# k-xlsx/huff-encoding

Hardware: AMD Instinct MI355X
Metric: encode+decode GB/s on 1 GiB bytes at 1/2/4/8 MI355X; % HBM roofline (higher is better)
Workload: dtype u8; 1 GPU; 1 GiB uniform bytes (BASELINE configs[1]), encode+decode, bit-exact; bytes_per_gpu=1073741824, global_bytes=1073741824, compressed_bytes_per_gpu=1073741824, parallelism=shard1

## Files before the change

### huff-encoding_amd/csrc/device/pack.hip

```cpp
#include "pack_emit.hpp"

namespace huff::dev {

namespace {

template <bool LONG>
constexpr int pack_waves() { return LONG ? 4 : static_cast<int>(kPackWaves); }
#ifndef HUFF_PACK_BPL
#define HUFF_PACK_BPL 16
#endif
#ifndef HUFF_PACK_AHEAD
#define HUFF_PACK_AHEAD 2
#endif
constexpr uint32_t kBPL = HUFF_PACK_BPL;
constexpr uint32_t kRoundB = 64 * kBPL;
constexpr int kAhead = HUFF_PACK_AHEAD;
static_assert(kBPL % 16 == 0, "lanes load whole 16-byte pieces");
static_assert(kBPL <= kIdx && kTaskSym % kRoundB == 0, "an index entry starts a lane; a task is whole rounds");
constexpr int kPieces = kBPL / 16;

struct LaneIn {
    uint4 v[kPieces];
};

#ifndef HUFF_PACK_COPIES
#define HUFF_PACK_COPIES 32
#endif
constexpr int kCopies = HUFF_PACK_COPIES;
template <bool LONG>
constexpr uint32_t table_words() { return 256u * kCopies * (LONG ? 2u : 1u); }

template <bool LONG, int G = 1>
__global__ __launch_bounds__(pack_waves<LONG>() * 64) void k_pack(PackArgs a) {
    constexpr int kWaves = pack_waves<LONG>();
    constexpr int kThreads = kWaves * 64;
    constexpr int C = kCopies;
    constexpr int LOGC = C == 32 ? 5 : C == 16 ? 4 : C == 8 ? 3 : -1;
    static_assert(LOGC > 0, "8, 16 or 32 table copies");
    using E = Entry<LONG>;
    using T = typename E::T;
    extern __shared__ __attribute__((aligned(16))) uint32_t lds[];
    T* tab = reinterpret_cast<T*>(lds);
    const uint32_t t = threadIdx.x, lane = t & 63, copy = t & (C - 1), wave = wave_index();
    uint32_t* stage = lds + table_words<LONG>() + wave * a.stage_words;

    const T* tg = reinterpret_cast<const T*>(LONG ? static_cast<const void*>(a.table.l) : static_cast<const void*>(a.table.s));
#pragma unroll 4
    for (int i = 0; i < 256 / (kThreads / C); ++i) {
        const uint32_t e = (t >> LOGC) + (kThreads / C) * i;
        tab[(e << LOGC) | copy] = tg[e];
    }
    for (uint32_t i = lane; i < a.stage_words; i += 64) stage[i] = 0;
    __syncthreads();

    for (uint32_t c = blockIdx.x * kWaves + wave; c < a.nchunks; c += a.grid * kWaves) {
        const uint64_t sym0 = static_cast<uint64_t>(c) * kChunk;
        const uint64_t nsym = (a.n - sym0 < kChunk) ? a.n - sym0 : kChunk;
        const uint64_t prev8 = (lane == 0 && sym0 >= 8) ? *reinterpret_cast<const uint64_t*>(a.in + sym0 - 8) : 0;
        const uint64_t cs = a.chunk_start[c];
        const uint64_t ce = a.chunk_start[c + 1];
        uint64_t stage_bit0 = (cs >> 7) << 7;
        const uint64_t own_lo = cs >> 3;
        const uint64_t own_hi = (c + 1 == a.nchunks) ? (ce + 7) >> 3 : ce >> 3;
        const uint32_t nrounds = static_cast<uint32_t>((nsym + kRoundB - 1) / kRoundB);
        const auto rin = buf_rsrc(a.in + sym0, static_cast<uint32_t>((nsym + 15) & ~15ull));

        auto load_round = [&](uint32_t r) {
            LaneIn x;
#pragma unroll
            for (int q = 0; q < kPieces; ++q) x.v[q] = buf_ld16(rin, r * kRoundB + lane * kBPL + 16 * q);
            return x;
        };
        LaneIn vq[kAhead];
#pragma unroll
        for (int i = 0; i < kAhead; ++i) vq[i] = load_round(i);

        if (lane == 0 && (cs & 7)) {
            const int64_t floor8 = static_cast<int64_t>(cs & ~7ull);
            int64_t pos = static_cast<int64_t>(cs);
            for (uint32_t k = 1; k <= 8 && pos > floor8; ++k) {
                uint8_t b;
                if (sym0 >= k) {
                    b = static_cast<uint8_t>(prev8 >> (8 * (8 - k)));
                } else {
                    const uint32_t j = k - static_cast<uint32_t>(sym0);
                    if (j > a.prev_tail_len) break;
                    b = a.prev_tail[8 - j];
                }
                const T ent = tab[static_cast<uint32_t>(b) << LOGC];
                const int64_t len = static_cast<int64_t>(ent & E::kMask);
                const uint64_t code = E::code(ent);
                if (len == 0) break;
                const int64_t start = pos - len;
                for (int64_t q = (start > floor8 ? start : floor8); q < pos; ++q) {
                    if ((code >> (pos - 1 - q)) & 1) {
                        const uint64_t sb = static_cast<uint64_t>(q) - stage_bit0;
                        stage[sb >> 5] |= 0x80000000u >> (sb & 31);
                    }
                }
                pos = start;
            }
        }
        wave_sync();

        uint64_t round_bit = cs, task_bit0 = cs;
        constexpr uint32_t kRoundsPerTask = kTaskSym / kRoundB;
        for (uint32_t r = 0; r < nrounds; ++r) {
            const LaneIn v = vq[0];
#pragma unroll
            for (int i = 0; i + 1 < kAhead; ++i) vq[i] = vq[i + 1];
            vq[kAhead - 1] = load_round(r + kAhead);
            const uint32_t s_in_chunk = r * kRoundB + lane * kBPL;
            const uint32_t nsym32 = static_cast<uint32_t>(nsym);
            const int nvalid = s_in_chunk >= nsym32 ? 0
                                                    : static_cast<int>(nsym32 - s_in_chunk < kBPL ? nsym32 - s_in_chunk : kBPL);

            uint32_t bits = 0;
            uint32_t wv[4 * kPieces];
#pragma unroll
            for (int q = 0; q < kPieces; ++q) {
                wv[4 * q] = v.v[q].x;
                wv[4 * q + 1] = v.v[q].y;
                wv[4 * q + 2] = v.v[q].z;
                wv[4 * q + 3] = v.v[q].w;
            }
            T ent[kBPL];
            auto lookup = [&](int k) -> T { return tab[(((wv[k >> 2] >> (8 * (k & 3))) & 0xFFu) << LOGC) | copy]; };
            if ((r + 1ull) * kRoundB <= nsym) {
#pragma unroll
                for (int k = 0; k < static_cast<int>(kBPL); ++k) ent[k] = lookup(k);
            } else {
#pragma unroll
                for (int k = 0; k < static_cast<int>(kBPL); ++k) ent[k] = (k < nvalid) ? lookup(k) : T(0);
            }
            uint32_t Lp[kBPL / 2];
            if constexpr (!LONG && G >= 2) {
#pragma unroll
                for (int k = 0; k < static_cast<int>(kBPL / 2); ++k) {
                    Lp[k] = len2(static_cast<uint32_t>(ent[2 * k]), static_cast<uint32_t>(ent[2 * k + 1]));
                    bits += Lp[k];
                }
            } else {
#pragma unroll
                for (int k = 0; k < static_cast<int>(kBPL); ++k) bits += static_cast<uint32_t>(ent[k] & E::kMask);
            }
            const uint32_t incl = wave_scan_incl(bits);
            const uint32_t tot = static_cast<uint32_t>(__builtin_amdgcn_readlane(static_cast<int>(incl), 63));
            const uint32_t excl = incl - bits;

            if (a.sub16) {
                if ((r % kRoundsPerTask) == 0) {
                    task_bit0 = round_bit;
                    if (lane == 0) a.task_base[(sym0 + r * kRoundB) / kTaskSym] = round_bit;
                }
                if (nvalid > 0 && (s_in_chunk & (kIdx - 1)) == 0)
                    a.sub16[(sym0 + s_in_chunk) / kIdx] = static_cast<uint16_t>(round_bit - task_bit0 + excl);
            } else if (a.sub_bit && nvalid > 0 && (s_in_chunk & (kIdx - 1)) == 0) {
                a.sub_bit[(sym0 + s_in_chunk) / kIdx] = static_cast<uint32_t>(round_bit - cs + excl);
            }

            if constexpr (LONG) {
                if (bits) emit_codes<LONG, static_cast<int>(kBPL)>(stage, round_bit - stage_bit0 + excl, ent);
            } else {
                emit_codes_or<G>(stage, static_cast<uint32_t>(round_bit - stage_bit0 + excl), ent, Lp);
            }
            wave_order();

            const uint64_t end_bit = round_bit + tot;
            const bool last = (r + 1 == nrounds);
            const uint32_t nseg_done = static_cast<uint32_t>((end_bit - stage_bit0) >> 7);
            const uint32_t nseg_store = last ? static_cast<uint32_t>((end_bit - stage_bit0 + 127) >> 7) : nseg_done;
            const uint64_t sb0 = stage_bit0 >> 3;
            const uint32_t full_lo = own_lo > sb0 ? static_cast<uint32_t>((own_lo - sb0 + 15) >> 4) : 0u;
            const uint64_t hi_rel = own_hi > sb0 ? (own_hi - sb0) >> 4 : 0;
            const uint32_t full_hi = static_cast<uint32_t>(hi_rel < 0x7FFFFFFFull ? hi_rel : 0x7FFFFFFFull);
            for (uint32_t s = lane; s < nseg_store; s += 64)
                store_segment(stage, s, sb0 + 16ull * s, full_lo, full_hi, own_lo, own_hi, a.out);
            const uint32_t used_words = static_cast<uint32_t>((end_bit - stage_bit0 + 31) >> 5);
            uint32_t keep = 0;
            if (!last && lane < 4) keep = stage[nseg_done * 4 + lane];
            wave_order();
            for (uint32_t i = lane; i < (used_words + 3) / 4; i += 64)
                reinterpret_cast<uint4*>(stage)[i] = make_uint4(0, 0, 0, 0);
            wave_order();
            if (!last) {
                if (lane < 4) stage[lane] = keep;
                stage_bit0 += static_cast<uint64_t>(nseg_done) << 7;
                wave_order();
            }
            round_bit = end_bit;
        }
    }
}

}

size_t pack_lds_bytes(bool long_codes, uint32_t max_len, uint32_t stage_words) {
    (void)max_len;
    const uint32_t table = long_codes ? table_words<true>() : table_words<false>();
    const uint32_t waves = long_codes ? pack_waves<true>() : pack_waves<false>();
    return static_cast<size_t>(table + waves * stage_words) * 4;
}

uint32_t pack_round_bytes() { return kRoundB; }

uint32_t pack_waves_per_group(bool long_codes) { return long_codes ? pack_waves<true>() : pack_waves<false>(); }

namespace {
using PackKern = void (*)(PackArgs);
PackKern pack_kernel(bool long_codes, uint32_t max_len) {
    if (long_codes) return k_pack<true>;
    if (max_len <= 8) return k_pack<false, 4>;
    if (max_len <= 16) return k_pack<false, 2>;
    return k_pack<false, 1>;
}
}

uint32_t pack_groups_per_cu(bool long_codes, uint32_t max_len, size_t lds) {
    int per = 0;
    const int threads = (long_codes ? pack_waves<true>() : pack_waves<false>()) * 64;
    if (hipOccupancyMaxActiveBlocksPerMultiprocessor(&per, pack_kernel(long_codes, max_len), threads, lds) !=
            hipSuccess ||
        per < 1) {
        const size_t by_lds = lds ? (160 * 1024) / lds : 8;
        per = static_cast<int>(by_lds < 1 ? 1 : by_lds > 8 ? 8 : by_lds);
    }
    return static_cast<uint32_t>(per);
}

hipError_t launch_pack(bool long_codes, const PackArgs& a, hipStream_t s) {
    if (a.nchunks == 0) return hipSuccess;
    const size_t lds = pack_lds_bytes(long_codes, a.max_len, a.stage_words);
    launch_k(pack_kernel(long_codes, a.max_len), dim3(a.grid),
             dim3((long_codes ? pack_waves<true>() : pack_waves<false>()) * 64), lds, s, a);
    return hipGetLastError();
}

}
```

### huff-encoding_amd/csrc/device/pack_emit.hpp

```cpp
#pragma once

#include "bitreader.hpp"

namespace huff::dev {

template <bool LONG>
struct Entry;
template <>
struct Entry<false> {
    using T = uint32_t;
    static constexpr uint32_t kMask = 31;
    __device__ static uint64_t code(T e) {
        const uint32_t len = e & 31u;
        return len ? e >> (32 - len) : 0u;
    }
};
template <>
struct Entry<true> {
    using T = uint64_t;
    static constexpr uint32_t kMask = 63;
    __device__ static uint64_t code(T e) { return e >> 6; }
};

template <bool LONG, int N>
__device__ __forceinline__ void emit_codes(uint32_t* __restrict__ stage, uint64_t p,
                                           const typename Entry<LONG>::T (&ent)[N]) {
    using E = Entry<LONG>;
    uint32_t w = static_cast<uint32_t>(p >> 5);
    uint32_t nacc = static_cast<uint32_t>(p & 31);
    bool shared_first = nacc != 0;
    uint64_t acc = 0;
    auto flush = [&]() {
        if (nacc >= 32) {
            const uint32_t word = static_cast<uint32_t>(acc >> (nacc - 32));
            if (shared_first) {
                __hip_atomic_fetch_or(&stage[w], word, __ATOMIC_RELAXED, __HIP_MEMORY_SCOPE_WORKGROUP);
                shared_first = false;
            } else {
                stage[w] = word;
            }
            ++w;
            nacc -= 32;
        }
    };
#pragma unroll
    for (int k = 0; k < N; ++k) {
        const uint32_t len = static_cast<uint32_t>(ent[k] & E::kMask);
        const uint64_t code = E::code(ent[k]);
        if (LONG && len > 32) {
            const uint32_t hl = len - 32;
            acc = (acc << hl) | (code >> 32);
            nacc += hl;
            flush();
            acc = (acc << 32) | (code & 0xFFFFFFFFull);
            nacc += 32;
            flush();
        } else {
            acc = (acc << len) | code;
            nacc += len;
            flush();
        }
    }
    if (nacc) {
        const uint32_t word = static_cast<uint32_t>(acc << (32 - nacc));
        __hip_atomic_fetch_or(&stage[w], word, __ATOMIC_RELAXED, __HIP_MEMORY_SCOPE_WORKGROUP);
    }
}

__device__ __forceinline__ uint32_t join2(uint32_t e0, uint32_t e1) {
    return (e0 & ~31u) | ((e1 & ~31u) >> (e0 & 31u));
}

__device__ __forceinline__ uint32_t len2(uint32_t e0, uint32_t e1) {
    uint32_t r;
    asm("v_add_u32_sdwa %0, %1, %2 dst_sel:DWORD dst_unused:UNUSED_PAD src0_sel:BYTE_0 src1_sel:BYTE_0"
        : "=v"(r)
        : "v"(e0), "v"(e1));
    return r;
}

template <int G, int N>
__device__ __forceinline__ void emit_codes_or(uint32_t* __restrict__ stage, uint32_t p, const uint32_t (&ent)[N],
                                              const uint32_t (&Lp)[N / 2]) {
    const uint32_t stage_addr = static_cast<uint32_t>(reinterpret_cast<uintptr_t>(
        (__attribute__((address_space(3))) uint32_t*)(stage)));
    uint32_t o = p;
#pragma unroll
    for (int k = 0; k < N; k += G) {
        uint32_t J, len;
        if constexpr (G == 1) {
            J = ent[k] & ~31u;
            len = ent[k] & 31u;
        } else if constexpr (G == 2) {
            J = join2(ent[k], ent[k + 1]);
            len = Lp[k / 2];
        } else {
            static_assert(G == 4, "groups of 1, 2 or 4 codes");
            const uint32_t l01 = Lp[k / 2];
            const uint32_t J23 = join2(ent[k + 2], ent[k + 3]);
            J = join2(ent[k], ent[k + 1]) | (J23 >> l01);
            len = l01 + Lp[k / 2 + 1];
        }
        const uint32_t s = o & 31u;
        uint32_t wa;
        asm volatile("v_lshl_add_u32 %0, %1, 2, %2" : "=v"(wa) : "v"(o >> 5), "v"(stage_addr));
        auto* w = (__attribute__((address_space(3))) uint32_t*)(static_cast<uintptr_t>(wa));
        __hip_atomic_fetch_or(w, J >> s, __ATOMIC_RELAXED, __HIP_MEMORY_SCOPE_WORKGROUP);
        __hip_atomic_fetch_or(w + 1, __builtin_amdgcn_alignbit(J, 0u, s), __ATOMIC_RELAXED,
                              __HIP_MEMORY_SCOPE_WORKGROUP);
        o += len;
    }
}

__device__ __forceinline__ void store_segment(const uint32_t* __restrict__ stage, uint32_t s, uint64_t gbyte,
                                              uint32_t full_lo, uint32_t full_hi, uint64_t own_lo, uint64_t own_hi,
                                              uint8_t* __restrict__ out) {
    uint4 v = reinterpret_cast<const uint4*>(stage)[s];
    v.x = __builtin_bswap32(v.x);
    v.y = __builtin_bswap32(v.y);
    v.z = __builtin_bswap32(v.z);
    v.w = __builtin_bswap32(v.w);
    if (s >= full_lo && s < full_hi) {
        *reinterpret_cast<uint4*>(out + gbyte) = v;
        return;
    }
    const uint32_t wv[4] = {v.x, v.y, v.z, v.w};
#pragma unroll
    for (int i = 0; i < 16; ++i) {
        const uint64_t g = gbyte + i;
        if (g >= own_lo && g < own_hi) out[g] = static_cast<uint8_t>(wv[i >> 2] >> (8 * (i & 3)));
    }
}

}
```

Before: 1276 GB/s.

## Rotate prefetch slots in place and clear stage while storing segments

The pack loop is restructured into an unrolled group of kAhead rounds. Each round consumes its own prefetch slot and refills it right after the table lookups, which avoids shifting the register queue every round. Stage words are now zeroed by the lane that stores each segment, and the carry words are moved inline, so a separate clearing pass and two wave barriers go away. Index writes use precomputed per-lane offsets and a running task-relative bit count. A byte-extract trick with an asm and empty asm barriers shape the schedule, at the cost of more code size and register pressure from the unrolled rounds.

```diff
diff --git a/huff-encoding_amd/csrc/device/pack.hip b/huff-encoding_amd/csrc/device/pack.hip
--- a/huff-encoding_amd/csrc/device/pack.hip
+++ b/huff-encoding_amd/csrc/device/pack.hip
@@ -16,7 +16,8 @@
 constexpr uint32_t kRoundB = 64 * kBPL;
 constexpr int kAhead = HUFF_PACK_AHEAD;
 static_assert(kBPL % 16 == 0, "lanes load whole 16-byte pieces");
-static_assert(kBPL <= kIdx && kTaskSym % kRoundB == 0, "an index entry starts a lane; a task is whole rounds");
+static_assert(kBPL <= kIdx && kIdx % kBPL == 0 && kRoundB % kIdx == 0 && kTaskSym % kRoundB == 0,
+              "an index entry starts a lane; a round is whole entries; a task is whole rounds");
 constexpr int kPieces = kBPL / 16;
 
 struct LaneIn {
@@ -46,10 +47,7 @@
 
     const T* tg = reinterpret_cast<const T*>(LONG ? static_cast<const void*>(a.table.l) : static_cast<const void*>(a.table.s));
 #pragma unroll 4
-    for (int i = 0; i < 256 / (kThreads / C); ++i) {
-        const uint32_t e = (t >> LOGC) + (kThreads / C) * i;
-        tab[(e << LOGC) | copy] = tg[e];
-    }
+    for (uint32_t e = t >> LOGC; e < 256; e += kThreads / C) tab[(e << LOGC) | copy] = tg[e];
     for (uint32_t i = lane; i < a.stage_words; i += 64) stage[i] = 0;
     __syncthreads();
 
@@ -103,36 +101,57 @@
         }
         wave_sync();
 
-        uint64_t round_bit = cs, task_bit0 = cs;
+        uint64_t round_bit = cs;
+        uint32_t task_rel = 0;
         constexpr uint32_t kRoundsPerTask = kTaskSym / kRoundB;
-        for (uint32_t r = 0; r < nrounds; ++r) {
-            const LaneIn v = vq[0];
-#pragma unroll
-            for (int i = 0; i + 1 < kAhead; ++i) vq[i] = vq[i + 1];
-            vq[kAhead - 1] = load_round(r + kAhead);
+        const uint32_t nsym32 = static_cast<uint32_t>(nsym);
+        const bool idx_lane = ((lane * kBPL) & (kIdx - 1)) == 0;
+        const uint32_t idx_off = lane * kBPL / kIdx;
+        const uint64_t idx0 = sym0 / kIdx;
+
+        auto loads_landed = [&] {
+#pragma unroll
+            for (int i = 0; i < kAhead; ++i)
+#pragma unroll
+                for (int q = 0; q < kPieces; ++q)
+                    asm volatile("" : "+v"(vq[i].v[q].x), "+v"(vq[i].v[q].y), "+v"(vq[i].v[q].z), "+v"(vq[i].v[q].w));
+        };
+        loads_landed();
+
+        auto round = [&](const uint32_t r, LaneIn& slot) {
             const uint32_t s_in_chunk = r * kRoundB + lane * kBPL;
-            const uint32_t nsym32 = static_cast<uint32_t>(nsym);
-            const int nvalid = s_in_chunk >= nsym32 ? 0
-                                                    : static_cast<int>(nsym32 - s_in_chunk < kBPL ? nsym32 - s_in_chunk : kBPL);
+            const bool whole = (r + 1) * kRoundB <= nsym32;
+            const bool live = whole || s_in_chunk < nsym32;
 
             uint32_t bits = 0;
             uint32_t wv[4 * kPieces];
 #pragma unroll
             for (int q = 0; q < kPieces; ++q) {
-                wv[4 * q] = v.v[q].x;
-                wv[4 * q + 1] = v.v[q].y;
-                wv[4 * q + 2] = v.v[q].z;
-                wv[4 * q + 3] = v.v[q].w;
+                wv[4 * q] = slot.v[q].x;
+                wv[4 * q + 1] = slot.v[q].y;
+                wv[4 * q + 2] = slot.v[q].z;
+                wv[4 * q + 3] = slot.v[q].w;
             }
             T ent[kBPL];
-            auto lookup = [&](int k) -> T { return tab[(((wv[k >> 2] >> (8 * (k & 3))) & 0xFFu) << LOGC) | copy]; };
-            if ((r + 1ull) * kRoundB <= nsym) {
+            auto lookup = [&](int k) -> T {
+                uint32_t b;
+                if ((k & 3) == 0)
+                    asm("v_and_b32 %0, 0xff, %1" : "=v"(b) : "v"(wv[k >> 2]));
+                else
+                    b = (wv[k >> 2] >> (8 * (k & 3))) & 0xFFu;
+                return tab[(b << LOGC) | copy];
+            };
+            if (whole) {
 #pragma unroll
                 for (int k = 0; k < static_cast<int>(kBPL); ++k) ent[k] = lookup(k);
             } else {
+                const int nvalid = s_in_chunk >= nsym32
+                                       ? 0
+                                       : static_cast<int>(nsym32 - s_in_chunk < kBPL ? nsym32 - s_in_chunk : kBPL);
 #pragma unroll
                 for (int k = 0; k < static_cast<int>(kBPL); ++k) ent[k] = (k < nvalid) ? lookup(k) : T(0);
             }
+            slot = load_round(r + kAhead);
             uint32_t Lp[kBPL / 2];
             if constexpr (!LONG && G >= 2) {
 #pragma unroll
@@ -150,13 +169,13 @@
 
             if (a.sub16) {
                 if ((r % kRoundsPerTask) == 0) {
-                    task_bit0 = round_bit;
+                    task_rel = 0;
                     if (lane == 0) a.task_base[(sym0 + r * kRoundB) / kTaskSym] = round_bit;
                 }
-                if (nvalid > 0 && (s_in_chunk & (kIdx - 1)) == 0)
-                    a.sub16[(sym0 + s_in_chunk) / kIdx] = static_cast<uint16_t>(round_bit - task_bit0 + excl);
-            } else if (a.sub_bit && nvalid > 0 && (s_in_chunk & (kIdx - 1)) == 0) {
-                a.sub_bit[(sym0 + s_in_chunk) / kIdx] = static_cast<uint32_t>(round_bit - cs + excl);
+                if (live && idx_lane)
+                    (a.sub16 + idx0 + r * (kRoundB / kIdx))[idx_off] = static_cast<uint16_t>(task_rel + excl);
+            } else if (a.sub_bit && live && idx_lane) {
+                (a.sub_bit + idx0 + r * (kRoundB / kIdx))[idx_off] = static_cast<uint32_t>(round_bit - cs) + excl;
             }
 
             if constexpr (LONG) {
@@ -165,6 +184,7 @@
                 emit_codes_or<G>(stage, static_cast<uint32_t>(round_bit - stage_bit0 + excl), ent, Lp);
             }
             wave_order();
+            loads_landed();
 
             const uint64_t end_bit = round_bit + tot;
             const bool last = (r + 1 == nrounds);
@@ -175,20 +195,23 @@
             const uint64_t hi_rel = own_hi > sb0 ? (own_hi - sb0) >> 4 : 0;
             const uint32_t full_hi = static_cast<uint32_t>(hi_rel < 0x7FFFFFFFull ? hi_rel : 0x7FFFFFFFull);
             for (uint32_t s = lane; s < nseg_store; s += 64)
-                store_segment(stage, s, sb0 + 16ull * s, full_lo, full_hi, own_lo, own_hi, a.out);
-            const uint32_t used_words = static_cast<uint32_t>((end_bit - stage_bit0 + 31) >> 5);
-            uint32_t keep = 0;
-            if (!last && lane < 4) keep = stage[nseg_done * 4 + lane];
+                store_segment<true>(stage, s, sb0 + 16ull * s, full_lo, full_hi, own_lo, own_hi, a.out);
+            if (!last) {
+                if (lane < 4) {
+                    const uint32_t keep = stage[nseg_done * 4 + lane];
+                    stage[nseg_done * 4 + lane] = 0;
+                    stage[lane] = keep;
+                }
+                stage_bit0 += static_cast<uint64_t>(nseg_done) << 7;
+            }
             wave_order();
-            for (uint32_t i = lane; i < (used_words + 3) / 4; i += 64)
-                reinterpret_cast<uint4*>(stage)[i] = make_uint4(0, 0, 0, 0);
-            wave_order();
-            if (!last) {
-                if (lane < 4) stage[lane] = keep;
-                stage_bit0 += static_cast<uint64_t>(nseg_done) << 7;
-                wave_order();
-            }
             round_bit = end_bit;
+            task_rel += tot;
+        };
+        for (uint32_t r0 = 0; r0 < nrounds; r0 += kAhead) {
+#pragma unroll
+            for (int i = 0; i < kAhead; ++i)
+                if (r0 + i < nrounds) round(r0 + i, vq[i]);
         }
     }
 }
diff --git a/huff-encoding_amd/csrc/device/pack_emit.hpp b/huff-encoding_amd/csrc/device/pack_emit.hpp
--- a/huff-encoding_amd/csrc/device/pack_emit.hpp
+++ b/huff-encoding_amd/csrc/device/pack_emit.hpp
@@ -112,10 +112,12 @@
     }
 }
 
-__device__ __forceinline__ void store_segment(const uint32_t* __restrict__ stage, uint32_t s, uint64_t gbyte,
+template <bool CLEAR = false>
+__device__ __forceinline__ void store_segment(uint32_t* __restrict__ stage, uint32_t s, uint64_t gbyte,
                                               uint32_t full_lo, uint32_t full_hi, uint64_t own_lo, uint64_t own_hi,
                                               uint8_t* __restrict__ out) {
     uint4 v = reinterpret_cast<const uint4*>(stage)[s];
+    if constexpr (CLEAR) reinterpret_cast<uint4*>(stage)[s] = make_uint4(0, 0, 0, 0);
     v.x = __builtin_bswap32(v.x);
     v.y = __builtin_bswap32(v.y);
     v.z = __builtin_bswap32(v.z);
```

After: 1261 GB/s. -1.2%, worse.
